# myungsub/meta-interpolation

Measured on AMD Instinct MI355X. Metric: inner-loop steps/sec, higher is better.
Workload: dtype f32 (3x3 convolutions: Winograd F(4x4) / F(2x2) on exact-f32 MFMAs, csrc/winograd4.h + winograd.hip; weight gradients and 5x5 / 7x7 / direct layers on csrc/convk*.hip: bf16x6 split operands, f32 accumulate; 51-tap op on 8-bit frames: exact integer frames x bf16x3 split taps, f32 accumulate); 1 GPU; c2_sepconv_256x448_b4_s5; plugin=sepconv, tasks_per_gpu=4, global_meta_batch=4, inner_steps=5, frame=256x448x3, inner_rule=lslr+SGD, seeded_weights=default, parallelism=task-parallel x1, 1 all-reduce of outer grads

## Files before the change

include/savfi_hip.h:

```cpp
#ifndef SAVFI_HIP_H_
#define SAVFI_HIP_H_

#include <stddef.h>
#include <stdint.h>

#ifdef __cplusplus
extern "C" {
#endif

#define SAVFI_ABI_VERSION 24

#define SAVFI_OK            0
#define SAVFI_E_NULL       (-1)
#define SAVFI_E_SHAPE      (-2)
#define SAVFI_E_UNSUPPORTED (-3)
#define SAVFI_E_TOOBIG     (-4)

int savfi_version(void);

int savfi_sepconv_fwd_f32(const float* in, const float* v, const float* h, float* out,
                          int B, int C, int Ho, int Wo, int K, void* stream);

int savfi_sepconv_bwd_f32(const float* in, const float* v, const float* h, const float* gO,
                          float* gI, float* gV, float* gH,
// ... 251 lines not shown
                              float* g1 , float* g2 , int N, int C, int H, int W, int md, void* stream);

int savfi_pwcwarp_fwd_f32(const float* img, const float* flow, float scale, float* out, int N, int C, int H, int W, void* stream);

int64_t savfi_bn_stats_scratch_floats(int N, int C, int H, int W, int n_per_group);
int savfi_bn_stats_f32(const float* x, float* mean, float* var, int64_t stat_stride, float* scratch , int N, int C, int H, int W,
                       int n_per_group, void* stream);
int savfi_bn_apply_relu_f32(const float* x, const float* mean, const float* var, int64_t stat_stride, const float* gamma ,
                            const float* beta , float eps, float* out, int N, int C, int H, int W, int n_per_group, int c_off,
                            int C_total, void* stream);
int savfi_bn_running_update_f32(int n, float* const* running, const float* const* stat, const int64_t* numel, const float* unbias,
                                float momentum, void* stream);

int savfi_maxpool2x2_f32(const float* in, float* out, int64_t planes, int H, int W, void* stream);

int savfi_upnearest2x_add_f32(const float* low, const float* skip, float* out, int64_t planes, int h, int w, int H, int W, void* stream);

int savfi_add_relu_f32(const float* a, const float* r, float* y, int64_t n, void* stream);

int savfi_charbonnier_f32(const float* a, const float* b, float* result, float* scratch, int rows, int64_t n, float eps, void* stream);
int savfi_charbonnier_bwd_f32(const float* a, const float* b, const float* g_loss, float* g_a, int rows, int64_t n, float eps,
                              void* stream);

#ifdef __cplusplus
}
#endif
#endif
```

meta-interpolation_amd/_hip.py:

```python
import ctypes
import os
import re
from ctypes import c_double, c_float, c_int, c_int64, c_void_p, POINTER

_PKG_DIR = os.path.dirname(os.path.abspath(__file__))
LIB_PATH = os.environ.get("SAVFI_HIP_LIB") or os.path.join(_PKG_DIR, "lib", "libsavfi_hip.so")
HEADER_PATH = os.path.join(os.path.dirname(_PKG_DIR), "include", "savfi_hip.h")

RULE_SGD, RULE_ADAM, RULE_ADAMAX_LSLR, RULE_ADAMAX_MSGD = 0, 1, 2, 3
LR_SCALAR, LR_ELEMENT = 0, 1
SSIM_RANGE_PER_ROW, SSIM_RANGE_BATCH, SSIM_RANGE_FIXED = 0, 1, 2
SEPCONV_PARTITION_WS, SEPCONV_PARTITION_X6, SEPCONV_PARTITION_FP32 = 0, 1, 2
ABI_VERSION = 24

_ERRORS = {-1: "SAVFI_E_NULL (a required pointer is NULL)",
           -2: "SAVFI_E_SHAPE (bad or inconsistent dimension)",
           -3: "SAVFI_E_UNSUPPORTED",
           -4: "SAVFI_E_TOOBIG (index arithmetic would overflow)"}


class SavfiHipError(RuntimeError):
    pass


# ... 116 lines not shown
    "savfi_upsample2x_window_bwd_masked_f32": [_P, _P, c_float, _P] + [c_int] * 12 + [_P],
    "savfi_upsample2x_bwd_form": [c_int, c_int, c_int],
    "savfi_bias_act_fwd_f32": [_P, _P, c_int, c_int, c_int, c_float, _P],
    "savfi_bias_act_scratch_floats": [c_int, c_int, c_int],
    "savfi_bias_act_bwd_f32": [_P, _P, _P, _P, _P, c_int, c_int, c_int, c_float, _P],
    "savfi_filterinterp_fwd_f32": [_P, _P, _P, _P] + [c_int] * 5 + [_P],
    "savfi_filterinterp_bwd_f32": [_P] * 7 + [c_int] * 5 + [_P],
    "savfi_filterinterp_fwd_slice_f32": [_P, _P, _P, _P] + [c_int] * 7 + [_P],
    "savfi_depthflowproj_scratch_bytes": [c_int, c_int, c_int],
    "savfi_depthflowproj_fwd_f32": [_P] * 5 + [c_int] * 4 + [_P],
    "savfi_depthflowproj_bwd_f32": [_P] * 7 + [c_int] * 3 + [_P],
    "savfi_correlation_fwd_f32": [_P, _P, _P] + [c_int] * 5 + [c_float, _P],
    "savfi_correlation_bwd_f32": [_P, _P, _P, _P, c_float, _P, _P] + [c_int] * 5 + [_P],
    "savfi_pwcwarp_fwd_f32": [_P, _P, c_float, _P] + [c_int] * 4 + [_P],
    "savfi_bn_stats_scratch_floats": [c_int] * 5,
    "savfi_bn_stats_f32": [_P, _P, _P, c_int64, _P] + [c_int] * 5 + [_P],
    "savfi_bn_apply_relu_f32": [_P, _P, _P, c_int64, _P, _P, c_float, _P] + [c_int] * 7 + [_P],
    "savfi_bn_running_update_f32": [c_int, _PP, _PP, _I64P, _FP, c_float, _P],
    "savfi_maxpool2x2_f32": [_P, _P, c_int64, c_int, c_int, _P],
    "savfi_upnearest2x_add_f32": [_P, _P, _P, c_int64, c_int, c_int, c_int, c_int, _P],
    "savfi_add_relu_f32": [_P, _P, _P, c_int64, _P],
    "savfi_charbonnier_f32": [_P, _P, _P, _P, c_int, c_int64, c_float, _P],
    "savfi_charbonnier_bwd_f32": [_P, _P, _P, _P, c_int, c_int64, c_float, _P],
}

_lib = None


def declared_symbols():
    with open(HEADER_PATH) as fh:
        text = fh.read()
    return sorted(set(re.findall(r"^\s*(?:int|int64_t)\s+(savfi_\w+)\s*\(", text, flags=re.M)))


def lib():
    global _lib
    if _lib is not None:
        return _lib
    if not os.path.exists(LIB_PATH):
        raise SavfiHipError(
            "%s is missing: build it with `python __graft_entry__.py build` "
            "(there is no CPU or PyTorch fallback for the savfi kernels)" % LIB_PATH)
    try:
        handle = ctypes.CDLL(LIB_PATH)
    except OSError as exc:
        raise SavfiHipError("cannot load %s: %s" % (LIB_PATH, exc))
# ... 133 lines not shown
```

meta-interpolation_amd/csrc/common.h:

```cpp
#pragma once
#include <hip/hip_runtime.h>
#include <stdint.h>
#include "savfi_hip.h"

#define SAVFI_WAVE 64


static inline int savfi_launch_status() {
  hipError_t e = hipGetLastError();
  return e == hipSuccess ? SAVFI_OK : (int)e;
}

static inline int savfi_cdiv(int64_t a, int64_t b) { return (int)((a + b - 1) / b); }

static inline int savfi_ensure_dynamic_lds(const void* kernel, size_t bytes, uint32_t& done_mask) {
  int dev = 0;
  if (hipGetDevice(&dev) != hipSuccess) return (int)hipGetLastError();
  const uint32_t bit = 1u << (dev & 31);
  if (__atomic_load_n(&done_mask, __ATOMIC_ACQUIRE) & bit) return SAVFI_OK;
  const hipError_t e = hipFuncSetAttribute(kernel, hipFuncAttributeMaxDynamicSharedMemorySize, (int)bytes);
  if (e != hipSuccess) return (int)e;
  __atomic_fetch_or(&done_mask, bit, __ATOMIC_RELEASE);
  return SAVFI_OK;
}

__device__ __forceinline__ float wave_sum(float x) {
#pragma unroll
  for (int off = 32; off > 0; off >>= 1) x += __shfl_xor(x, off, SAVFI_WAVE);
  return x;
}

template <int NW>
__device__ __forceinline__ float block_sum(float x, float* lds ) {
  x = wave_sum(x);
  const int lane = threadIdx.x & (SAVFI_WAVE - 1), wid = threadIdx.x / SAVFI_WAVE;
  if (lane == 0) lds[wid] = x;
  __syncthreads();
  float t = (threadIdx.x < NW) ? lds[threadIdx.x] : 0.f;
  if (wid == 0) t = wave_sum(t);
  __syncthreads();
  return t;
}

__device__ __forceinline__ float savfi_quantize255(float x) {
  const float v = x * 255.f;
  const float c = v < 0.f ? 0.f : (v > 255.f ? 255.f : v);
  return rintf(c);
// ... 15 lines not shown
```

meta-interpolation_amd/csrc/convk_wgrad.hip:

```cpp
#include "common.h"
#include <stdlib.h>
#include <algorithm>

typedef float f32x4 __attribute__((ext_vector_type(4)));
typedef short bf16x8 __attribute__((ext_vector_type(8)));
typedef short bf16x4 __attribute__((ext_vector_type(4)));
typedef unsigned u32x4 __attribute__((ext_vector_type(4)));
typedef int i32x4 __attribute__((ext_vector_type(4)));
__device__ float ckw_raw_buffer_load_f32(i32x4 rsrc, int voffset, int soffset, int aux) __asm("llvm.amdgcn.raw.buffer.load.f32");

namespace {

constexpr int WG_THREADS = 256;
constexpr int UR = 4, UW = 32;

__device__ __forceinline__ i32x4 ckw_rsrc(const void* base, unsigned bytes) {
  const unsigned long long p = reinterpret_cast<unsigned long long>(base);
  i32x4 r;
  r.x = (int)(unsigned)p;
  r.y = (int)(unsigned)(p >> 32);
  r.z = (int)bytes;
  r.w = 0x00020000;
  return r;
}
// ... 716 lines not shown
  a.N = N; a.T = T; a.Ci = Ci; a.Co = Co; a.H = H; a.W = W; a.pad = pad; a.reflect = reflect ? 1 : 0;
  a.Ho = H + 2 * pad - K + 1; a.Wo = W + 2 * pad - K + 1;
  a.cobs = p.cobs; a.cibs = p.cibs; a.splits = p.splits; a.units = p.units; a.units_per_split = p.ups_per_split;
  a.upr = p.upr; a.ups = p.ups;
  const int blocks = T * p.cobs * p.cibs * p.splits;
  hipStream_t st = (hipStream_t)stream;
  float* bias_partial = gb ? workspace + (size_t)p.splits * T * Co * Ci * K * K : nullptr;
  if (p.form == 2) rc = launch_wgrad3_ring(a, blocks, bias_partial, st);
  else if (K == 3 && precise) rc = p.mt == 4 ? launch_wgrad<3, 4, 1, true>(a, blocks, st) : launch_wgrad<3, 2, 1, true>(a, blocks, st);
  else if (K == 3 && p.ng == 2) rc = launch_wgrad<3, 4, 1, false, 2>(a, blocks, st);
  else if (K == 3) rc = p.mt == 4 ? launch_wgrad<3, 4, 1>(a, blocks, st) : p.nt == 2 ? launch_wgrad<3, 2, 2>(a, blocks, st) : launch_wgrad<3, 2, 1>(a, blocks, st);
  else if (K == 5) rc = precise ? launch_wgrad<5, 2, 1, true>(a, blocks, st) : p.nt == 2 ? launch_wgrad<5, 2, 2>(a, blocks, st) : launch_wgrad<5, 2, 1>(a, blocks, st);
  else rc = launch_wgrad<7, 2, 1>(a, blocks, st);
  if (rc != SAVFI_OK) return rc;
  const long long n = (long long)T * Co * Ci * K * K;
  const bool v4 = n % 4 == 0 && (((uintptr_t)workspace | (uintptr_t)gw) & 15u) == 0;
  const long long nb = gb ? (long long)T * Co : 0;
  const unsigned main_blocks = (unsigned)(v4 ? (n / 4 + 31) / 32 : (n + 31) / 32), bias_blocks = (unsigned)((nb + 31) / 32);
  if (v4) hipLaunchKernelGGL(convk_wgrad_reduce<true>, dim3(main_blocks + bias_blocks), dim3(256), 0, st, workspace, gw, n, p.splits, main_blocks, bias_partial, gb, nb);
  else hipLaunchKernelGGL(convk_wgrad_reduce<false>, dim3(main_blocks + bias_blocks), dim3(256), 0, st, workspace, gw, n, p.splits, main_blocks, bias_partial, gb, nb);
  return savfi_launch_status();
}
}
```

meta-interpolation_amd/csrc/wgrad.hip:

```cpp
#include "common.h"

namespace {

typedef float f32x4 __attribute__((ext_vector_type(4)));

constexpr int GNT = 256;
constexpr int GCO = 32, GCI = 32, GSEG = 64;
constexpr int GP = 68;
constexpr int G_FLOATS = GCO * GP;
constexpr int X_FLOATS = 3 * GCI * GP;
constexpr int BUF_FLOATS = G_FLOATS + X_FLOATS;
constexpr int TILE_FLOATS = 2 * 2 * 9 * 256;
constexpr int LDS_FLOATS_G = (2 * BUF_FLOATS > TILE_FLOATS) ? 2 * BUF_FLOATS : TILE_FLOATS;

struct WgradArgs {
  const float* x;
  const float* gz;
  float* partial;
  int Ci, Co, H, W, Ho, Wo, pad, rows, nseg, nrowchunk, cibs;
  int T;
};

struct Staged {
  float g[8], x[3][8], halo;
// ... 614 lines not shown
           bias_partial};
  if (gb) hipLaunchKernelGGL(wino_wgrad3x3<true>, dim3(p.nsplit, p.cobs * p.cibs, T), dim3(256), lds_bias, st, a);
  else hipLaunchKernelGGL(wino_wgrad3x3<false>, dim3(p.nsplit, p.cobs * p.cibs, T), dim3(256), lds, st, a);
  if (int e = savfi_launch_status()) return e;
  if (gb) {
    hipLaunchKernelGGL(wino_wgrad_bias_reduce, dim3(savfi_cdiv(Co, 64), T), dim3(64), 0, st, bias_partial, gb, Co, p.cobs, p.nsplit);
    if (int e = savfi_launch_status()) return e;
  }
  const int ntiles = p.cobs * p.cibs;
  const size_t block_floats = (size_t)ntiles * WW_BLOCK_FLOATS;
  float* stage2 = workspace + p.partial_floats;
  if (p.ngroups == 1) {
    hipLaunchKernelGGL(wino_wgrad_reduce2, dim3(savfi_cdiv(Co * Ci * 9, 256), T), dim3(256), 0, st, workspace, gw, Co, Ci, p.cibs, ntiles,
                       p.nsplit);
    return savfi_launch_status();
  }
  hipLaunchKernelGGL(wgrad_reduce1, dim3((unsigned)((block_floats / 4 + 255) / 256), p.ngroups, T), dim3(256), 0, st, workspace,
                     stage2, block_floats, p.nsplit);
  if (int e = savfi_launch_status()) return e;
  hipLaunchKernelGGL(wino_wgrad_reduce2, dim3(savfi_cdiv(Co * Ci * 9, 256), T), dim3(256), 0, st, stage2, gw, Co, Ci, p.cibs, ntiles,
                     p.ngroups);
  return savfi_launch_status();
}
```

meta-interpolation_amd/csrc/winograd.hip:

```cpp
#include "common.h"
#include <type_traits>

typedef float f32x4 __attribute__((ext_vector_type(4)));
typedef int i32x4 __attribute__((ext_vector_type(4)));
__device__ f32x4 savfi_raw_buffer_load_x4(i32x4 rsrc, int voffset, int soffset, int aux) __asm("llvm.amdgcn.raw.buffer.load.v4f32");
typedef float f32x2 __attribute__((ext_vector_type(2)));
__device__ void savfi_raw_buffer_store_x2(f32x2 data, i32x4 rsrc, int voffset, int soffset, int aux) __asm("llvm.amdgcn.raw.buffer.store.v2f32");
__device__ f32x2 savfi_raw_buffer_load_x2(i32x4 rsrc, int voffset, int soffset, int aux) __asm("llvm.amdgcn.raw.buffer.load.v2f32");
__device__ float savfi_raw_buffer_load_x1(i32x4 rsrc, int voffset, int soffset, int aux) __asm("llvm.amdgcn.raw.buffer.load.f32");
__device__ void savfi_raw_buffer_store_x1(float data, i32x4 rsrc, int voffset, int soffset, int aux) __asm("llvm.amdgcn.raw.buffer.store.f32");
__device__ void savfi_raw_buffer_store_x4(f32x4 data, i32x4 rsrc, int voffset, int soffset, int aux) __asm("llvm.amdgcn.raw.buffer.store.v4f32");

namespace {

#include "winograd4.h"

constexpr int WNT = 256;
constexpr int TILES_WG = 64;
constexpr int COB = 32;
constexpr int CIB = 4;
#ifndef WINO_VS
#define WINO_VS 80
#endif
constexpr int VS = WINO_VS;
// ... 471 lines not shown
  if (e >= total) return;
  float acc = 0.f;
  for (int s = 0; s < nsplit; ++s) acc += partial[(size_t)s * total + e];
  if (bias) {
    const size_t plane = e / HW;
    acc += bias[((plane / I) % T) * I + plane % I];
  }
  acc = acc > 0.f ? acc : slope * acc;
  if (mask) acc = mask[e] > 0.f ? acc : acc * mask_slope;
  out[e] = acc;
}

int round_up(int v, int m) { return (v + m - 1) / m * m; }

#ifndef SAVFI_WINO_SPLIT_SLOTS
#define SAVFI_WINO_SPLIT_SLOTS 512
#endif

struct WinoPlan {
  int K, I, KP, IP, off, Ho, Wo, th, tw, tile_shift, nsplit, chunks_per_split;
  int ty4, tx4;
  int64_t u_floats, partial_floats;
  bool f4;
};

inline bool f4_for(int K, int I, int form) { return form != 2 && w4::use_f4(K, I); }
inline int kp_for(int K, int I, int form) { return f4_for(K, I, form) ? w4::kp_of(K) : (K + 2 * CIB - 1) / (2 * CIB) * (2 * CIB); }
inline int ip_for(int K, int I, int form) { return f4_for(K, I, form) ? w4::ip_of(I) : (I + COB - 1) / COB * COB; }
inline int64_t u_floats_for(int K, int I, int form) { return (int64_t)(f4_for(K, I, form) ? w4::PTS : 16) * kp_for(K, I, form) * ip_for(K, I, form); }

bool make_plan(WinoPlan& p, int N, int Ci, int Co, int H, int W, int pad, int mode) {
  const int form = (mode & 2) ? 2 : 0;
  mode &= 1;
  p.K = mode == 0 ? Ci : Co;
  p.I = mode == 0 ? Co : Ci;
  p.f4 = f4_for(p.K, p.I, form);
  p.KP = kp_for(p.K, p.I, form);
  p.IP = ip_for(p.K, p.I, form);
  p.off = mode == 0 ? pad : 2 - pad;
  p.Ho = H + 2 * p.off - 2;
  p.Wo = W + 2 * p.off - 2;
  if (p.Ho <= 0 || p.Wo <= 0) return false;
  if (p.f4) {
    const int ty4 = savfi_cdiv(p.Ho, 4), tx4 = savfi_cdiv(p.Wo, 4);
    int64_t best4 = -1;
#ifndef SAVFI_W4_TS_ORDER
#define SAVFI_W4_TS_ORDER 2
// ... 2 lines not shown
    for (int s : {3, 4, 2, 5, 1, 0}) {
#elif SAVFI_W4_TS_ORDER == 1
    for (int s : {4, 3, 5, 2, 1, 0}) {
#else
    for (int s : {5, 4, 3, 2, 1, 0}) {
#endif
      const int64_t blocks = (int64_t)savfi_cdiv(ty4, w4::TT >> s) * savfi_cdiv(tx4, 1 << s);
      if (best4 < 0 || blocks < best4) { best4 = blocks; p.tile_shift = s; }
    }
    p.th = savfi_cdiv(ty4, w4::TT >> p.tile_shift);
    p.tw = savfi_cdiv(tx4, 1 << p.tile_shift);
    p.ty4 = ty4;
    p.tx4 = tx4;
    const int nchunk4 = p.KP / w4::KC;
    const int64_t wgs4 = (int64_t)p.th * p.tw * (p.IP / w4::COB) * N;
    int want4 = (int)(SAVFI_WINO_SPLIT_SLOTS / (wgs4 > 0 ? wgs4 : 1));
    want4 = (want4 < 2 || nchunk4 < 32) ? 1 : (want4 > 8 ? 8 : want4);
    int cps4 = savfi_cdiv(nchunk4, want4);
    if (cps4 < 8) cps4 = nchunk4 < 8 ? nchunk4 : 8;
    p.chunks_per_split = cps4;
    p.nsplit = savfi_cdiv(nchunk4, cps4);
    p.u_floats = u_floats_for(p.K, p.I, form);
    p.partial_floats = p.nsplit > 1 ? (int64_t)p.nsplit * N * p.I * p.Ho * p.Wo : 0;
    return true;
  }
  const int ty = savfi_cdiv(p.Ho, 2), tx = savfi_cdiv(p.Wo, 2);
  int64_t best = -1;
  for (int s : {4, 3, 5, 2}) {
    const int64_t blocks = (int64_t)savfi_cdiv(ty, TILES_WG >> s) * savfi_cdiv(tx, 1 << s);
    if (best < 0 || blocks < best) { best = blocks; p.tile_shift = s; }
  }
  p.th = savfi_cdiv(ty, TILES_WG >> p.tile_shift);
  p.tw = savfi_cdiv(tx, 1 << p.tile_shift);
  const int nchunk = p.KP / CIB;
  const int64_t wgs = (int64_t)p.th * p.tw * (p.IP / COB) * N;
  constexpr int slots = SAVFI_WINO_SPLIT_SLOTS;
  int want = (int)(slots / wgs);
  want = want < 1 ? 1 : (want > 8 ? 8 : want);
  int cps = round_up(savfi_cdiv(nchunk, want), 2);
  if (cps < 8) cps = nchunk < 8 ? nchunk : 8;
  p.chunks_per_split = cps;
  p.nsplit = savfi_cdiv(nchunk, cps);
  if (SAVFI_WINO_SPLIT_SLOTS == 0) { p.nsplit = 1; p.chunks_per_split = nchunk; }
  p.u_floats = (int64_t)16 * p.KP * p.IP;
  p.partial_floats = p.nsplit > 1 ? (int64_t)p.nsplit * N * p.I * p.Ho * p.Wo : 0;
  return true;
}



}

#ifdef WINO_TRACE
static unsigned long long* g_trace = nullptr;
static size_t g_trace_wgs = 0;
static unsigned long long* savfi_wino_trace_buffer(size_t wgs) {
  if (!g_trace) (void)hipMalloc(&g_trace, (size_t)(1 << 20) * 64);
  g_trace_wgs = wgs;
  return g_trace;
}
extern "C" int savfi_debug_wino_trace(unsigned long long* host, long long cap) {
  (void)hipDeviceSynchronize();
  const size_t n = g_trace_wgs < (size_t)cap ? g_trace_wgs : (size_t)cap;
  (void)hipMemcpy(host, g_trace, n * 64, hipMemcpyDeviceToHost);
  return (int)n;
}
#endif

// ... 16 lines not shown
static int w4_block_decode = 0;
static int64_t w4_tile_groups(const WinoPlan& p) {
  return w4_block_decode ? (int64_t)p.th * p.tw : ((int64_t)p.ty4 * p.tx4 + w4::TT - 1) / w4::TT;
}
extern "C" int64_t savfi_conv3x3_f4_launched_workgroups(int N, int Ci, int Co, int H, int W, int pad, int mode) {
  if (N <= 0 || Ci <= 0 || Co <= 0 || H <= 0 || W <= 0) return SAVFI_E_SHAPE;
  if ((mode & ~3) || (pad != 0 && pad != 1)) return SAVFI_E_UNSUPPORTED;
  WinoPlan p;
  if (!make_plan(p, N, Ci, Co, H, W, pad, mode)) return SAVFI_E_SHAPE;
  return p.f4 ? w4_tile_groups(p) * (p.IP / w4::COB) * p.nsplit * N : 0;
}
extern "C" int savfi_conv3x3_debug_f4_block_decode(int on, int* previous) {
  if (previous) *previous = w4_block_decode;
  w4_block_decode = on ? 1 : 0;
  return SAVFI_OK;
}

extern "C" int64_t savfi_conv3x3_workspace_floats(int N, int Ci, int Co, int H, int W, int pad, int mode) {
  return savfi_conv3x3_tasks_workspace_floats(N, 1, Ci, Co, H, W, pad, mode);
}

namespace {

template <int VECW, int IN16, bool MASK, bool POOL = false>
int launch_wino4(const w4::W4Args& a4, int64_t wgs4, hipStream_t st) {
  static uint32_t configured = 0;
  constexpr size_t lds4 = (size_t)w4::LDS_FLOATS * sizeof(float);
  auto kern = w4::wino4_conv3x3<VECW, IN16, MASK, POOL>;
  if (int rc = savfi_ensure_dynamic_lds(reinterpret_cast<const void*>(kern), lds4, configured)) return rc;
  hipLaunchKernelGGL(kern, dim3((unsigned)wgs4), dim3(256), lds4, st, a4);
  return savfi_launch_status();
}

bool pools_in_epilogue(const WinoPlan& p, int mode) {
  return p.f4 && (mode & 1) == 0 && p.nsplit == 1 && p.Wo % 2 == 0 && p.Ho >= 2;
}

int launch_conv(const WinoPlan& p, const float* x, const float* U, const float* bias, float* out, float* partial, int N, int T,
                int H, int W, int mode, float slope, hipStream_t st, const float* mask = nullptr, float mask_slope = 1.f,
                int out_unit16 = 0, int in_unit16 = 0, float* pooled = nullptr) {
  if (pooled && (!pools_in_epilogue(p, mode) || mask || out_unit16 || in_unit16)) return SAVFI_E_UNSUPPORTED;
  if (p.f4) {
    const int64_t ntb = w4_tile_groups(p);
    const int64_t wgs4 = ntb * (p.IP / w4::COB) * p.nsplit * N;
    if (wgs4 > 0x7fffffffLL || T > 65535) return SAVFI_E_TOOBIG;
    if (mask && (out_unit16 || in_unit16)) return SAVFI_E_UNSUPPORTED;
    if (p.nsplit > 1 && (out_unit16 || in_unit16 || !partial)) return SAVFI_E_UNSUPPORTED;
    if (in_unit16 && ((p.off != 1 && p.off != 2) || p.Wo % 2 != 0)) return SAVFI_E_UNSUPPORTED;
    w4::W4Args a4{x, U, (mode & 1) == 0 ? bias : nullptr, out, p.K, p.I, p.KP, p.IP, H, W, p.Ho, p.Wo, p.off, p.th, p.tw, slope,
                  p.tile_shift, T, N, p.nsplit > 1 ? nullptr : mask, mask_slope, out_unit16, p.nsplit, p.chunks_per_split, partial,
                  w4_block_decode ? 0 : 1, p.ty4, p.tx4, (int)ntb, p.tx4 > 1 ? (unsigned)(0x100000000ull / (unsigned)p.tx4) : 0xffffffffu,
                  pooled, p.Ho / 2, p.Wo / 2};
    const int vecw = p.Wo % 4 == 0 ? 4 : (p.Wo % 2 == 0 ? 2 : 1);
    auto go = [&](auto kern) { return kern(a4, wgs4, st); };
    if (pooled) return vecw == 4 ? go(launch_wino4<4, 0, false, true>) : go(launch_wino4<2, 0, false, true>);
    if (in_unit16 && p.off == 1) return vecw == 4 ? go(launch_wino4<4, 2, false>) : go(launch_wino4<2, 2, false>);
    if (in_unit16) return vecw == 4 ? go(launch_wino4<4, 3, false>) : go(launch_wino4<2, 3, false>);
    if (p.nsplit > 1) {
      const int rc = vecw == 4 ? go(launch_wino4<4, 0, false>) : vecw == 2 ? go(launch_wino4<2, 0, false>) : go(launch_wino4<1, 0, false>);
      if (rc != SAVFI_OK) return rc;
      const size_t total = (size_t)N * p.I * p.Ho * p.Wo;
      hipLaunchKernelGGL(wino_split_reduce, dim3((unsigned)((total + 255) / 256)), dim3(256), 0, st, partial, (mode & 1) == 0 ? bias : nullptr, out,
                         p.nsplit, total, p.I, p.Ho * p.Wo, slope, T, mask, mask_slope);
      return savfi_launch_status();
    }
    if (mask) return vecw == 4 ? go(launch_wino4<4, 0, true>) : vecw == 2 ? go(launch_wino4<2, 0, true>) : go(launch_wino4<1, 0, true>);
    return vecw == 4 ? go(launch_wino4<4, 0, false>) : vecw == 2 ? go(launch_wino4<2, 0, false>) : go(launch_wino4<1, 0, false>);
  }
  const int64_t wgs = (int64_t)p.th * p.tw * (p.IP / COB) * p.nsplit * N;
  if (wgs > 0x7fffffffLL || T > 65535) return SAVFI_E_TOOBIG;
  constexpr size_t lds = (size_t)LDS_FLOATS * sizeof(float);
  const float* b = (mode & 1) == 0 ? bias : nullptr;
  WinoArgs a{x, U, b, out, p.K, p.I, p.KP, p.IP, H, W, p.Ho, p.Wo, p.off, p.th, p.tw, slope, p.tile_shift, p.nsplit,
             p.chunks_per_split, partial, T, N, mask, mask_slope, out_unit16
#ifdef WINO_TRACE
             , savfi_wino_trace_buffer((size_t)wgs)
#endif
  };
  if (in_unit16) hipLaunchKernelGGL((wino_conv3x3<true, true>), dim3((unsigned)wgs), dim3(WNT), lds, st, a);
  else if (p.Wo % 2 == 0) hipLaunchKernelGGL(wino_conv3x3<true>, dim3((unsigned)wgs), dim3(WNT), lds, st, a);
// ... 164 lines not shown
  if (!in_unit16_ok(p, H, W)) return SAVFI_E_UNSUPPORTED;
  return launch_conv(p, gy, u, nullptr, gx, nullptr, N, T, H, W, 1, 1.f, (hipStream_t)stream, nullptr, 1.f, 0, 1);
}

extern "C" int savfi_conv3x3_dgrad_masked_form_f32(const float* gy, const float* u, const float* mask, float mask_slope, float* gx,
                                                   float* workspace, int N, int T, int Ci, int Co, int H, int W, int pad, int form,
                                                   void* stream) {
  if (!gy || !u || !gx || !mask) return SAVFI_E_NULL;
  if (form != 0 && form != 2) return SAVFI_E_UNSUPPORTED;
  WinoPlan p;
  if (int e = check_conv_args(p, N, T, Ci, Co, H, W, pad, 1 | form)) return e;
  if (p.partial_floats > 0 && !workspace) return SAVFI_E_NULL;
  return launch_conv(p, gy, u, nullptr, gx, workspace, N, T, H, W, 1, 1.f, (hipStream_t)stream, mask, mask_slope);
}
extern "C" int savfi_conv3x3_dgrad_masked_f32(const float* gy, const float* u, const float* mask, float mask_slope, float* gx,
                                              float* workspace, int N, int T, int Ci, int Co, int H, int W, int pad, void* stream) {
  return savfi_conv3x3_dgrad_masked_form_f32(gy, u, mask, mask_slope, gx, workspace, N, T, Ci, Co, H, W, pad, 0, stream);
}

extern "C" int savfi_conv3x3_f32(const float* x, const float* w, const float* bias, float* out, float* workspace,
                                 int N, int Ci, int Co, int H, int W, int pad, int mode, float slope, void* stream) {
  return savfi_conv3x3_tasks_f32(x, w, bias, out, workspace, N, 1, Ci, Co, H, W, pad, mode, slope, stream);
}
```

meta-interpolation_amd/csrc/winograd4.h:

```cpp
#pragma once

namespace w4 {

constexpr int TT = 32;
constexpr int COB = 32;
constexpr int KC = 8;
constexpr int PTS = 36;
constexpr int VBUF = PTS * KC * TT;
constexpr int XBUF = PTS * 16 * TT;
constexpr int LDS_FLOATS = XBUF > 2 * VBUF ? XBUF : 2 * VBUF;
#ifndef SAVFI_W4_MAXC
#define SAVFI_W4_MAXC 512
#endif

__host__ __device__ inline bool use_f4(int K, int I) { return K <= SAVFI_W4_MAXC && I <= SAVFI_W4_MAXC; }
__host__ __device__ inline int kp_of(int K) { return (K + KC - 1) / KC * KC; }
__host__ __device__ inline int ip_of(int I) { return (I + COB - 1) / COB * COB; }

__device__ __forceinline__ void g_rows(const float (&g)[3], float (&t)[6]) {
  const float s = g[0] + g[2];
  const float s4 = fmaf(4.f, g[2], g[0]);
  t[0] = 0.25f * g[0];
  t[1] = (s + g[1]) * (-1.f / 6.f);
  t[2] = (s - g[1]) * (-1.f / 6.f);
// ... 56 lines not shown
    float* dst = U + ((((size_t)chunk * ncob + cobq) * 4 + wv) * 2 + s2) * (18 * 64) + off;
    *reinterpret_cast<f32x4*>(dst) = *reinterpret_cast<const f32x4*>(stage + e);
  }
}

struct W4Args {
  const float* x;
  const float* U;
  const float* bias;
  float* out;
  int K, I, KP, IP, H, W, Ho, Wo, off, tiles_y, tiles_x;
  float slope;
  int tile_shift;
  int T, N;
  const float* mask;
  float mask_slope;
  int out_unit16;
  int nsplit, chunks_per_split;
  float* partial;
  int flat, ty4, tx4, ntb;
  unsigned tx_mul;
  float* pooled;
  int Hp, Wp;
};

__device__ __forceinline__ i32x4 w4_rsrc(const void* base, unsigned bytes) {
  const unsigned long long p = reinterpret_cast<unsigned long long>(base);
  i32x4 r;
  r.x = (int)(unsigned)p;
  r.y = (int)(unsigned)(p >> 32);
  r.z = (int)bytes;
  r.w = 0x00020000;
  return r;
}

__device__ __forceinline__ i32x4 w4_uniform(i32x4 r) {
  r.x = __builtin_amdgcn_readfirstlane(r.x); r.y = __builtin_amdgcn_readfirstlane(r.y);
  r.z = __builtin_amdgcn_readfirstlane(r.z); r.w = __builtin_amdgcn_readfirstlane(r.w);
  return r;
}

__device__ __forceinline__ void bt6(float d0, float d1, float d2, float d3, float d4, float d5, float (&o)[6]) {
  const float a = fmaf(-4.f, d2, d4), b = fmaf(-4.f, d1, d3);
  const float c = d4 - d2, e = d3 - d1;
  o[0] = fmaf(4.f, d0, fmaf(-5.f, d2, d4));
  o[1] = a + b;
// ... 11 lines not shown
  o[1] = a + b;
  o[2] = a - b;
  o[3] = w4_fma2(2.f, e, c);
  o[4] = w4_fma2(-2.f, e, c);
  o[5] = w4_fma2(4.f, d1, w4_fma2(-5.f, d3, d5));
}

__device__ __forceinline__ void at6(float m0, float m1, float m2, float m3, float m4, float m5, float (&o)[4]) {
  const float s1 = m1 + m2, d1 = m1 - m2, s2 = m3 + m4, d2 = m3 - m4;
  o[0] = m0 + s1 + s2;
  o[1] = fmaf(2.f, d2, d1);
  o[2] = fmaf(4.f, s2, s1);
  o[3] = fmaf(8.f, d2, d1) + m5;
}

__device__ __forceinline__ void at6p(f32x2 m0, f32x2 m1, f32x2 m2, f32x2 m3, f32x2 m4, f32x2 m5, f32x2 (&o)[4]) {
  const f32x2 s1 = m1 + m2, d1 = m1 - m2, s2 = m3 + m4, d2 = m3 - m4;
  o[0] = m0 + s1 + s2;
  o[1] = w4_fma2(2.f, d2, d1);
  o[2] = w4_fma2(4.f, s2, s1);
  o[3] = w4_fma2(8.f, d2, d1) + m5;
}

template <int VECW, int IN16, bool MASK, bool POOL = false>
__global__ __launch_bounds__(256, 2) void wino4_conv3x3(W4Args a) {
  extern __shared__ __attribute__((aligned(16))) float lds[];
  const int tid = threadIdx.x, lane = tid & 63, w = __builtin_amdgcn_readfirstlane(tid >> 6);
  const int j = lane & 15, kg = lane >> 4;

  const int nblk = a.IP / COB;
  int tb, cob, n, sp;
  {
    const unsigned flat = blockIdx.x, nwg = gridDim.x;
    const unsigned ntb = (unsigned)a.ntb;
    const unsigned xcd = flat & 7u, q8 = nwg >> 3, rem = nwg & 7u;
    unsigned item = xcd * q8 + min(xcd, rem) + (flat >> 3);
    cob = (int)(item % (unsigned)nblk);
    item /= (unsigned)nblk;
    tb = (int)(item % ntb);
    item /= ntb;
    sp = (int)(item % (unsigned)a.nsplit);
    n = (int)(item / (unsigned)a.nsplit);
  }
  const int i0 = cob * COB;
  const int task = a.T > 1 ? n % a.T : 0;
  const size_t cplane = (size_t)a.H * a.W;
  const float* xp = a.x + (size_t)n * a.K * cplane;
// ... 290 lines not shown
#pragma unroll
          for (int e = 0; e < NS; ++e) {
            if constexpr (VECW == 4) {
              const f32x4 v = savfi_raw_buffer_load_x4(mrs, (int)ooff[r][e], 0, 0);
              mk[MASK ? ch : 0][r][0] = v.x; mk[MASK ? ch : 0][r][1] = v.y; mk[MASK ? ch : 0][r][2] = v.z; mk[MASK ? ch : 0][r][3] = v.w;
            } else if constexpr (VECW == 2) {
              const f32x2 v = savfi_raw_buffer_load_x2(mrs, (int)ooff[r][e], 0, 0);
              mk[MASK ? ch : 0][r][2 * e] = v.x; mk[MASK ? ch : 0][r][2 * e + 1] = v.y;
            } else {
              mk[MASK ? ch : 0][r][e] = savfi_raw_buffer_load_x1(mrs, (int)ooff1(r, e), 0, 0);
            }
          }
      }
    }
  };
  auto by_wave = [&](auto&& f) {
    switch (w) {
      case 0: f(std::integral_constant<int, 0>{}); break;
      case 1: f(std::integral_constant<int, 1>{}); break;
      case 2: f(std::integral_constant<int, 2>{}); break;
      default: f(std::integral_constant<int, 3>{}); break;
    }
  };
  f32x2* const xl = reinterpret_cast<f32x2*>(lds) + olane;
  const float slope = a.slope;
  auto put = [&](auto cb_tag) {
    constexpr int cb = decltype(cb_tag)::value;
    by_wave([&](auto wtag) {
      constexpr int WV = decltype(wtag)::value;
#pragma unroll
      for (int q = 0; q < 9; ++q)
#pragma unroll
        for (int p = 0; p < 4; ++p)
          if (p != WV) xl[((9 * WV + q) * 4 + p) * 64] = (f32x2){acc[q][cb][p >> 1][2 * (p & 1)], acc[q][cb][p >> 1][2 * (p & 1) + 1]};
    });
  };
  auto gather = [&](auto cb_tag, f32x2 (&t4)[4][6]) {
    constexpr int cb = decltype(cb_tag)::value;
    by_wave([&](auto wtag) {
      constexpr int WV = decltype(wtag)::value;
#pragma unroll
      for (int c = 0; c < 6; ++c) {
        f32x2 m[6], o[4];
#pragma unroll
        for (int r = 0; r < 6; ++r) {
          const int xi = 6 * r + c, wp = xi / 9, q = xi % 9;
// ... 13 lines not shown
#pragma unroll
      for (int ch = 0; ch < 2; ++ch) {
        const float b = bvals[cb][ch];
        const int i = i0 + 16 * cb + 4 * okg + 2 * oh + ch;
        const i32x4 ors = w4_uniform(a.out_unit16 ? w4_rsrc(obase + (size_t)n * a.I * a.Ho * a.Wo, (unsigned)a.I * oplane) : wave_rsrc(obase, cb, ch, oplane));
        const unsigned choff = a.out_unit16 ? (i < a.I ? (unsigned)i * 64u : 0x40000000u) : 0u;
        i32x4 prs = ors;
        if constexpr (POOL) prs = w4_uniform(wave_rsrc(a.pooled, cb, ch, pplane));
        float ye[4];
#pragma unroll
        for (int r = 0; r < 4; ++r) {
          float y[4];
          at6(t4[r][0][ch], t4[r][1][ch], t4[r][2][ch], t4[r][3][ch], t4[r][4][ch], t4[r][5][ch], y);
#pragma unroll
          for (int c = 0; c < 4; ++c) {
            float v = y[c];
            if constexpr (ACT >= 1) v += b;
            if constexpr (ACT == 2) v = fmaxf(v, 0.f);
            if constexpr (ACT == 3) v = fmaxf(v, 0.f) + slope * fminf(v, 0.f);
            if constexpr (MASK) v = mk[MASK ? ch : 0][r][c] > 0.f ? v : v * a.mask_slope;
            y[c] = v;
          }
          if constexpr (VECW == 4) {
            savfi_raw_buffer_store_x4((f32x4){y[0], y[1], y[2], y[3]}, ors, (int)(ooff[r][0] + choff), 0, 0);
          } else if constexpr (VECW == 2) {
            savfi_raw_buffer_store_x2((f32x2){y[0], y[1]}, ors, (int)(ooff[r][0] + choff), 0, 0);
            savfi_raw_buffer_store_x2((f32x2){y[2], y[3]}, ors, (int)(ooff[r][1] + choff), 0, 0);
          } else {
#pragma unroll
            for (int c = 0; c < 4; ++c) savfi_raw_buffer_store_x1(y[c], ors, (int)(ooff1(r, c) + choff), 0, 0);
          }
          if constexpr (POOL) {
            if (r % 2 == 0) {
#pragma unroll
              for (int c = 0; c < 4; ++c) ye[c] = y[c];
            } else {
              const float p0 = (((ye[0] + ye[1]) + y[0]) + y[1]) / 4.f, p1 = (((ye[2] + ye[3]) + y[2]) + y[3]) / 4.f;
              if constexpr (VECW == 4) {
                savfi_raw_buffer_store_x2((f32x2){p0, p1}, prs, (int)poff[r >> 1][0], 0, 0);
              } else {
                savfi_raw_buffer_store_x1(p0, prs, (int)poff[r >> 1][0], 0, 0);
                savfi_raw_buffer_store_x1(p1, prs, (int)poff[r >> 1][PS - 1], 0, 0);
              }
            }
          }
        }
      }
    };
    if (slope == 1.f || split) {
      if (a.bias == nullptr || split) finish(std::integral_constant<int, 0>{});
      else finish(std::integral_constant<int, 1>{});
    } else if (slope == 0.f) {
      finish(std::integral_constant<int, 2>{});
    } else {
      finish(std::integral_constant<int, 3>{});
    }
  };
  using R0 = std::integral_constant<int, 0>;
  using R1 = std::integral_constant<int, 1>;
  f32x2 t4[4][6];
  fetch_mask(0);
  put(R0{});
  __syncthreads();
  gather(R0{}, t4);
  store(R0{}, t4);
  fetch_mask(1);
  __syncthreads();
  put(R1{});
  __syncthreads();
  gather(R1{}, t4);
  store(R1{}, t4);
}

}
```

Before: 253.2 inner-loop steps/sec.

## Fuse split-K partial reduction into Winograd F4 conv via ticket-based last-block combine

Adds a per-stream ticket buffer so that, when the F(4x4) Winograd conv splits the channel reduction across workgroups, the last workgroup to finish a tile sums all split partials and applies bias, activation and mask in place. This removes the separate combine kernel launch and its extra pass over the partial buffer. In exchange each workgroup now does an atomic ticket draw with fences, and the last one does a serial reduction. Stores use a cache-policy bit, and an optional pre-read mode warms the partials.

```diff
diff --git a/include/savfi_hip.h b/include/savfi_hip.h
--- a/include/savfi_hip.h
+++ b/include/savfi_hip.h
@@ -297,6 +297,15 @@
 int savfi_charbonnier_bwd_f32(const float* a, const float* b, const float* g_loss, float* g_a, int rows, int64_t n, float eps,
                               void* stream);
 
+#define SAVFI_SPLIT_FAMILY_WINO_WGRAD  0
+#define SAVFI_SPLIT_FAMILY_WINO_CONV   1
+#define SAVFI_SPLIT_FAMILY_CONVK_WGRAD 2
+int savfi_set_split_combine(int mode);
+int savfi_get_split_combine(void);
+int savfi_split_combine_prepare(void* stream);
+int savfi_split_combine_tickets(void* stream, unsigned* out, int n);
+int savfi_split_combine_form(int family, int N, int T, int Ci, int Co, int H, int W, int K, int pad, int mode, int* splits);
+
 #ifdef __cplusplus
 }
 #endif
diff --git a/meta-interpolation_amd/_hip.py b/meta-interpolation_amd/_hip.py
--- a/meta-interpolation_amd/_hip.py
+++ b/meta-interpolation_amd/_hip.py
@@ -162,6 +162,11 @@
     "savfi_add_relu_f32": [_P, _P, _P, c_int64, _P],
     "savfi_charbonnier_f32": [_P, _P, _P, _P, c_int, c_int64, c_float, _P],
     "savfi_charbonnier_bwd_f32": [_P, _P, _P, _P, c_int, c_int64, c_float, _P],
+    "savfi_set_split_combine": [c_int],
+    "savfi_get_split_combine": [],
+    "savfi_split_combine_prepare": [_P],
+    "savfi_split_combine_tickets": [_P, _P, c_int],
+    "savfi_split_combine_form": [c_int] * 10 + [_P],
 }
 
 _lib = None
diff --git a/meta-interpolation_amd/csrc/common.h b/meta-interpolation_amd/csrc/common.h
--- a/meta-interpolation_amd/csrc/common.h
+++ b/meta-interpolation_amd/csrc/common.h
@@ -23,6 +23,90 @@
   __atomic_fetch_or(&done_mask, bit, __ATOMIC_RELEASE);
   return SAVFI_OK;
 }
+
+constexpr int SAVFI_TICKET_WORDS = 1 << 16;
+unsigned* savfi_split_combine_acquire(hipStream_t st, int* mode);
+void savfi_split_combine_launch_failed(hipStream_t st);
+int savfi_wino_wgrad_combine_form(int N, int T, int Ci, int Co, int H, int W, int pad, int* splits);
+int savfi_wino_conv_combine_form(int N, int T, int Ci, int Co, int H, int W, int pad, int mode, int* splits);
+int savfi_convk_wgrad_combine_form(int N, int T, int Ci, int Co, int H, int W, int K, int pad, int* splits);
+
+#ifdef __HIPCC__
+__device__ __forceinline__ bool savfi_ticket_draw(unsigned* tickets, unsigned tile, unsigned splits, unsigned* flag) {
+  asm volatile("s_waitcnt vmcnt(0)" ::: "memory");
+  __syncthreads();
+  if (threadIdx.x == 0) {
+    const unsigned drawn = __hip_atomic_fetch_add(tickets + tile, 1u, __ATOMIC_RELAXED, __HIP_MEMORY_SCOPE_AGENT);
+    const unsigned last = drawn == splits - 1u ? 1u : 0u;
+    if (last) {
+      __builtin_amdgcn_fence(__ATOMIC_ACQUIRE, "agent");
+      asm volatile("s_waitcnt vmcnt(0)" ::: "memory");
+    }
+    *flag = last;
+  }
+  __syncthreads();
+  return __builtin_amdgcn_readfirstlane(*reinterpret_cast<volatile unsigned*>(flag)) != 0u;
+}
+template <int V, int NI, typename BiasOf>
+__device__ __forceinline__ void savfi_split_finish_rows(const float* partial, size_t total, int nsplit, const unsigned (&e)[NI], unsigned ok,
+                                                        BiasOf&& bias_of, bool has_bias, float slope, const float* mask, float mask_slope,
+                                                        float* out, bool write) {
+  typedef float fv __attribute__((ext_vector_type(V)));
+  fv acc[NI];
+#pragma unroll
+  for (int k = 0; k < NI; ++k) acc[k] = (fv)(0.f);
+  int s = 0;
+  for (; s + 1 < nsplit; s += 2) {
+    const float* p0 = partial + (size_t)s * total;
+    const float* p1 = p0 + total;
+    fv v0[NI], v1[NI];
+#pragma unroll
+    for (int k = 0; k < NI; ++k) v0[k] = *reinterpret_cast<const fv*>(p0 + e[k]);
+#pragma unroll
+    for (int k = 0; k < NI; ++k) v1[k] = *reinterpret_cast<const fv*>(p1 + e[k]);
+#pragma unroll
+    for (int k = 0; k < NI; ++k) acc[k] += v0[k];
+#pragma unroll
+    for (int k = 0; k < NI; ++k) acc[k] += v1[k];
+  }
+  if (s < nsplit) {
+    const float* p0 = partial + (size_t)s * total;
+    fv v0[NI];
+#pragma unroll
+    for (int k = 0; k < NI; ++k) v0[k] = *reinterpret_cast<const fv*>(p0 + e[k]);
+#pragma unroll
+    for (int k = 0; k < NI; ++k) acc[k] += v0[k];
+  }
+  if (!write) {
+#pragma unroll
+    for (int k = 0; k < NI; ++k)
+#pragma unroll
+      for (int q = 0; q < V; ++q) asm volatile("" ::"v"(acc[k][q]));
+    return;
+  }
+  fv mv[NI];
+  if (mask) {
+#pragma unroll
+    for (int k = 0; k < NI; ++k) mv[k] = *reinterpret_cast<const fv*>(mask + e[k]);
+  }
+#pragma unroll
+  for (int k = 0; k < NI; ++k) {
+    const float b = has_bias ? bias_of(k) : 0.f;
+#pragma unroll
+    for (int q = 0; q < V; ++q) {
+      float a = acc[k][q];
+      if (has_bias) a += b;
+      a = a > 0.f ? a : slope * a;
+      if (mask) a = mv[k][q] > 0.f ? a : a * mask_slope;
+      acc[k][q] = a;
+    }
+    if (ok >> k & 1u) *reinterpret_cast<fv*>(out + e[k]) = acc[k];
+  }
+}
+__device__ __forceinline__ void savfi_ticket_reset(unsigned* tickets, unsigned tile) {
+  if (threadIdx.x == 0) __hip_atomic_store(tickets + tile, 0u, __ATOMIC_RELAXED, __HIP_MEMORY_SCOPE_AGENT);
+}
+#endif
 
 __device__ __forceinline__ float wave_sum(float x) {
 #pragma unroll
diff --git a/meta-interpolation_amd/csrc/convk_wgrad.hip b/meta-interpolation_amd/csrc/convk_wgrad.hip
--- a/meta-interpolation_amd/csrc/convk_wgrad.hip
+++ b/meta-interpolation_amd/csrc/convk_wgrad.hip
@@ -762,3 +762,11 @@
   return savfi_launch_status();
 }
 }
+
+int savfi_convk_wgrad_combine_form(int N, int T, int Ci, int Co, int H, int W, int K, int pad, int* splits) {
+  WgPlan p;
+  const int rc = wg_plan(p, N, T, Ci, Co, H, W, K, pad, false);
+  if (rc != SAVFI_OK) return rc;
+  *splits = p.splits;
+  return 0;
+}
diff --git a/meta-interpolation_amd/csrc/split_combine.hip b/meta-interpolation_amd/csrc/split_combine.hip
--- /dev/null
+++ b/meta-interpolation_amd/csrc/split_combine.hip
@@ -0,0 +1,125 @@
+#include "common.h"
+#include <mutex>
+#include <vector>
+
+#ifndef SAVFI_SPLIT_COMBINE
+#define SAVFI_SPLIT_COMBINE 1
+#endif
+
+namespace {
+
+struct TicketBlock {
+  int dev;
+  hipStream_t stream;
+  unsigned* words;
+  bool dirty;
+};
+std::mutex g_lock;
+std::vector<TicketBlock> g_blocks;
+int g_mode = SAVFI_SPLIT_COMBINE;
+
+bool stream_is_capturing(hipStream_t st) {
+  hipStreamCaptureStatus cs = hipStreamCaptureStatusNone;
+  if (hipStreamIsCapturing(st, &cs) != hipSuccess) { (void)hipGetLastError(); return true; }
+  return cs != hipStreamCaptureStatusNone;
+}
+
+TicketBlock* find_block(int dev, hipStream_t st) {
+  for (TicketBlock& b : g_blocks)
+    if (b.dev == dev && b.stream == st) return &b;
+  return nullptr;
+}
+
+unsigned* block_for(hipStream_t st) {
+  int dev = 0;
+  if (hipGetDevice(&dev) != hipSuccess) { (void)hipGetLastError(); return nullptr; }
+  TicketBlock* b = find_block(dev, st);
+  if (b && !b->dirty) return b->words;
+  if (stream_is_capturing(st)) return nullptr;
+  if (!b) {
+    unsigned* words = nullptr;
+    if (hipMalloc(reinterpret_cast<void**>(&words), (size_t)SAVFI_TICKET_WORDS * sizeof(unsigned)) != hipSuccess) {
+      (void)hipGetLastError();
+      return nullptr;
+    }
+    g_blocks.push_back(TicketBlock{dev, st, words, true});
+    b = &g_blocks.back();
+  }
+  if (hipMemsetAsync(b->words, 0, (size_t)SAVFI_TICKET_WORDS * sizeof(unsigned), st) != hipSuccess) {
+    (void)hipGetLastError();
+    return nullptr;
+  }
+  b->dirty = false;
+  return b->words;
+}
+
+}
+
+unsigned* savfi_split_combine_acquire(hipStream_t st, int* mode) {
+  std::lock_guard<std::mutex> hold(g_lock);
+  *mode = g_mode;
+  return g_mode == 0 ? nullptr : block_for(st);
+}
+
+void savfi_split_combine_launch_failed(hipStream_t st) {
+  std::lock_guard<std::mutex> hold(g_lock);
+  int dev = 0;
+  if (hipGetDevice(&dev) != hipSuccess) { (void)hipGetLastError(); return; }
+  if (TicketBlock* b = find_block(dev, st)) b->dirty = true;
+}
+
+extern "C" int savfi_set_split_combine(int mode) {
+  if (mode < 0 || mode > 2) return SAVFI_E_UNSUPPORTED;
+  std::lock_guard<std::mutex> hold(g_lock);
+  g_mode = mode;
+  return SAVFI_OK;
+}
+
+extern "C" int savfi_get_split_combine(void) {
+  std::lock_guard<std::mutex> hold(g_lock);
+  return g_mode;
+}
+
+extern "C" int savfi_split_combine_prepare(void* stream) {
+  std::lock_guard<std::mutex> hold(g_lock);
+  return block_for((hipStream_t)stream) ? SAVFI_OK : SAVFI_E_UNSUPPORTED;
+}
+
+extern "C" int savfi_split_combine_tickets(void* stream, unsigned* out, int n) {
+  if (!out) return SAVFI_E_NULL;
+  if (n <= 0 || n > SAVFI_TICKET_WORDS) return SAVFI_E_SHAPE;
+  hipStream_t st = (hipStream_t)stream;
+  unsigned* words = nullptr;
+  {
+    std::lock_guard<std::mutex> hold(g_lock);
+    int dev = 0;
+    if (hipGetDevice(&dev) != hipSuccess) return (int)hipGetLastError();
+    if (TicketBlock* b = find_block(dev, st)) words = b->words;
+  }
+  if (!words) return SAVFI_E_UNSUPPORTED;
+  if (hipMemcpyAsync(out, words, (size_t)n * sizeof(unsigned), hipMemcpyDeviceToHost, st) != hipSuccess) return (int)hipGetLastError();
+  if (hipStreamSynchronize(st) != hipSuccess) return (int)hipGetLastError();
+  return SAVFI_OK;
+}
+
+extern "C" int savfi_split_combine_form(int family, int N, int T, int Ci, int Co, int H, int W, int K, int pad, int mode, int* splits) {
+  int sp = 0;
+  int rc;
+  switch (family) {
+    case SAVFI_SPLIT_FAMILY_WINO_WGRAD:
+      if (K != 3) return SAVFI_E_UNSUPPORTED;
+      rc = savfi_wino_wgrad_combine_form(N, T, Ci, Co, H, W, pad, &sp);
+      break;
+    case SAVFI_SPLIT_FAMILY_WINO_CONV:
+      if (K != 3) return SAVFI_E_UNSUPPORTED;
+      rc = savfi_wino_conv_combine_form(N, T, Ci, Co, H, W, pad, mode, &sp);
+      break;
+    case SAVFI_SPLIT_FAMILY_CONVK_WGRAD:
+      rc = savfi_convk_wgrad_combine_form(N, T, Ci, Co, H, W, K, pad, &sp);
+      break;
+    default:
+      return SAVFI_E_UNSUPPORTED;
+  }
+  if (rc >= 0 && splits) *splits = sp;
+  return rc;
+}
diff --git a/meta-interpolation_amd/csrc/wgrad.hip b/meta-interpolation_amd/csrc/wgrad.hip
--- a/meta-interpolation_amd/csrc/wgrad.hip
+++ b/meta-interpolation_amd/csrc/wgrad.hip
@@ -660,3 +660,12 @@
                      p.ngroups);
   return savfi_launch_status();
 }
+
+int savfi_wino_wgrad_combine_form(int N, int T, int Ci, int Co, int H, int W, int pad, int* splits) {
+  if (N <= 0 || T <= 0 || N % T != 0 || Ci <= 0 || Co <= 0 || H <= 0 || W <= 0) return SAVFI_E_SHAPE;
+  if (pad != 0 && pad != 1) return SAVFI_E_UNSUPPORTED;
+  WWPlan p;
+  if (!ww_plan(p, N, T, Ci, Co, H, W, pad)) return SAVFI_E_SHAPE;
+  *splits = p.nsplit;
+  return 0;
+}
diff --git a/meta-interpolation_amd/csrc/winograd.hip b/meta-interpolation_amd/csrc/winograd.hip
--- a/meta-interpolation_amd/csrc/winograd.hip
+++ b/meta-interpolation_amd/csrc/winograd.hip
@@ -517,7 +517,16 @@
   int ty4, tx4;
   int64_t u_floats, partial_floats;
   bool f4;
+  bool combine;
 };
+
+#ifndef SAVFI_WINO4_COMBINE_KB
+#define SAVFI_WINO4_COMBINE_KB 128
+#endif
+inline bool wino_combines(bool f4, int nsplit, int64_t tiles, int64_t out_floats) {
+  return f4 && nsplit > 1 && (int64_t)nsplit * 64 <= SAVFI_WINO4_COMBINE_KB && tiles <= SAVFI_TICKET_WORDS &&
+         out_floats < ((int64_t)1 << 31);
+}
 
 inline bool f4_for(int K, int I, int form) { return form != 2 && w4::use_f4(K, I); }
 inline int kp_for(int K, int I, int form) { return f4_for(K, I, form) ? w4::kp_of(K) : (K + 2 * CIB - 1) / (2 * CIB) * (2 * CIB); }
@@ -566,6 +575,7 @@
     p.nsplit = savfi_cdiv(nchunk4, cps4);
     p.u_floats = u_floats_for(p.K, p.I, form);
     p.partial_floats = p.nsplit > 1 ? (int64_t)p.nsplit * N * p.I * p.Ho * p.Wo : 0;
+    p.combine = wino_combines(true, p.nsplit, wgs4, (int64_t)N * p.I * p.Ho * p.Wo);
     return true;
   }
   const int ty = savfi_cdiv(p.Ho, 2), tx = savfi_cdiv(p.Wo, 2);
@@ -588,6 +598,7 @@
   if (SAVFI_WINO_SPLIT_SLOTS == 0) { p.nsplit = 1; p.chunks_per_split = nchunk; }
   p.u_floats = (int64_t)16 * p.KP * p.IP;
   p.partial_floats = p.nsplit > 1 ? (int64_t)p.nsplit * N * p.I * p.Ho * p.Wo : 0;
+  p.combine = wino_combines(false, p.nsplit, wgs, (int64_t)N * p.I * p.Ho * p.Wo);
   return true;
 }
 
@@ -650,11 +661,11 @@
 
 namespace {
 
-template <int VECW, int IN16, bool MASK, bool POOL = false>
+template <int VECW, int IN16, bool MASK, bool POOL = false, bool COMBINE = false>
 int launch_wino4(const w4::W4Args& a4, int64_t wgs4, hipStream_t st) {
   static uint32_t configured = 0;
   constexpr size_t lds4 = (size_t)w4::LDS_FLOATS * sizeof(float);
-  auto kern = w4::wino4_conv3x3<VECW, IN16, MASK, POOL>;
+  auto kern = w4::wino4_conv3x3<VECW, IN16, MASK, POOL, COMBINE>;
   if (int rc = savfi_ensure_dynamic_lds(reinterpret_cast<const void*>(kern), lds4, configured)) return rc;
   hipLaunchKernelGGL(kern, dim3((unsigned)wgs4), dim3(256), lds4, st, a4);
   return savfi_launch_status();
@@ -678,12 +689,23 @@
     w4::W4Args a4{x, U, (mode & 1) == 0 ? bias : nullptr, out, p.K, p.I, p.KP, p.IP, H, W, p.Ho, p.Wo, p.off, p.th, p.tw, slope,
                   p.tile_shift, T, N, p.nsplit > 1 ? nullptr : mask, mask_slope, out_unit16, p.nsplit, p.chunks_per_split, partial,
                   w4_block_decode ? 0 : 1, p.ty4, p.tx4, (int)ntb, p.tx4 > 1 ? (unsigned)(0x100000000ull / (unsigned)p.tx4) : 0xffffffffu,
-                  pooled, p.Ho / 2, p.Wo / 2};
+                  pooled, p.Ho / 2, p.Wo / 2, nullptr, mask, 0};
     const int vecw = p.Wo % 4 == 0 ? 4 : (p.Wo % 2 == 0 ? 2 : 1);
     auto go = [&](auto kern) { return kern(a4, wgs4, st); };
     if (pooled) return vecw == 4 ? go(launch_wino4<4, 0, false, true>) : go(launch_wino4<2, 0, false, true>);
     if (in_unit16 && p.off == 1) return vecw == 4 ? go(launch_wino4<4, 2, false>) : go(launch_wino4<2, 2, false>);
     if (in_unit16) return vecw == 4 ? go(launch_wino4<4, 3, false>) : go(launch_wino4<2, 3, false>);
+    if (p.nsplit > 1 && p.combine && ((((uintptr_t)partial | (uintptr_t)out | (uintptr_t)mask) & 15u) == 0)) {
+      int cmode = 0;
+      a4.tickets = savfi_split_combine_acquire(st, &cmode);
+      if (a4.tickets) {
+        a4.pre_read = cmode == 2;
+        const int rc = vecw == 4 ? go(launch_wino4<4, 0, false, false, true>)
+                                 : vecw == 2 ? go(launch_wino4<2, 0, false, false, true>) : go(launch_wino4<1, 0, false, false, true>);
+        if (rc > 0) savfi_split_combine_launch_failed(st);
+        return rc;
+      }
+    }
     if (p.nsplit > 1) {
       const int rc = vecw == 4 ? go(launch_wino4<4, 0, false>) : vecw == 2 ? go(launch_wino4<2, 0, false>) : go(launch_wino4<1, 0, false>);
       if (rc != SAVFI_OK) return rc;
@@ -894,3 +916,10 @@
                                  int N, int Ci, int Co, int H, int W, int pad, int mode, float slope, void* stream) {
   return savfi_conv3x3_tasks_f32(x, w, bias, out, workspace, N, 1, Ci, Co, H, W, pad, mode, slope, stream);
 }
+
+int savfi_wino_conv_combine_form(int N, int T, int Ci, int Co, int H, int W, int pad, int mode, int* splits) {
+  WinoPlan p;
+  if (int rc = check_conv_args(p, N, T, Ci, Co, H, W, pad, mode)) return rc;
+  *splits = p.nsplit;
+  return p.combine ? 1 : 0;
+}
diff --git a/meta-interpolation_amd/csrc/winograd4.h b/meta-interpolation_amd/csrc/winograd4.h
--- a/meta-interpolation_amd/csrc/winograd4.h
+++ b/meta-interpolation_amd/csrc/winograd4.h
@@ -102,6 +102,9 @@
   unsigned tx_mul;
   float* pooled;
   int Hp, Wp;
+  unsigned* tickets;
+  const float* rmask;
+  int pre_read;
 };
 
 __device__ __forceinline__ i32x4 w4_rsrc(const void* base, unsigned bytes) {
@@ -159,7 +162,7 @@
   o[3] = w4_fma2(8.f, d2, d1) + m5;
 }
 
-template <int VECW, int IN16, bool MASK, bool POOL = false>
+template <int VECW, int IN16, bool MASK, bool POOL = false, bool COMBINE = false>
 __global__ __launch_bounds__(256, 2) void wino4_conv3x3(W4Args a) {
   extern __shared__ __attribute__((aligned(16))) float lds[];
   const int tid = threadIdx.x, lane = tid & 63, w = __builtin_amdgcn_readfirstlane(tid >> 6);
@@ -496,6 +499,7 @@
       default: f(std::integral_constant<int, 3>{}); break;
     }
   };
+  constexpr int OAUX = COMBINE ? 16 : 0;
   f32x2* const xl = reinterpret_cast<f32x2*>(lds) + olane;
   const float slope = a.slope;
   auto put = [&](auto cb_tag) {
@@ -555,13 +559,13 @@
             y[c] = v;
           }
           if constexpr (VECW == 4) {
-            savfi_raw_buffer_store_x4((f32x4){y[0], y[1], y[2], y[3]}, ors, (int)(ooff[r][0] + choff), 0, 0);
+            savfi_raw_buffer_store_x4((f32x4){y[0], y[1], y[2], y[3]}, ors, (int)(ooff[r][0] + choff), 0, OAUX);
           } else if constexpr (VECW == 2) {
-            savfi_raw_buffer_store_x2((f32x2){y[0], y[1]}, ors, (int)(ooff[r][0] + choff), 0, 0);
-            savfi_raw_buffer_store_x2((f32x2){y[2], y[3]}, ors, (int)(ooff[r][1] + choff), 0, 0);
+            savfi_raw_buffer_store_x2((f32x2){y[0], y[1]}, ors, (int)(ooff[r][0] + choff), 0, OAUX);
+            savfi_raw_buffer_store_x2((f32x2){y[2], y[3]}, ors, (int)(ooff[r][1] + choff), 0, OAUX);
           } else {
 #pragma unroll
-            for (int c = 0; c < 4; ++c) savfi_raw_buffer_store_x1(y[c], ors, (int)(ooff1(r, c) + choff), 0, 0);
+            for (int c = 0; c < 4; ++c) savfi_raw_buffer_store_x1(y[c], ors, (int)(ooff1(r, c) + choff), 0, OAUX);
           }
           if constexpr (POOL) {
             if (r % 2 == 0) {
@@ -603,6 +607,37 @@
   __syncthreads();
   gather(R1{}, t4);
   store(R1{}, t4);
-}
-
-}
+  if constexpr (COMBINE) {
+    const size_t total = (size_t)a.N * a.I * a.Ho * a.Wo;
+    constexpr int UPR = 4 / VECW, UNITS = COB * TT * 4 * UPR, NI = VECW == 4 ? 8 : 16;
+    static_assert(UNITS % (256 * NI) == 0, "whole batches");
+    auto finish_tile = [&](bool write) {
+#pragma unroll 1
+      for (int u0 = tid; u0 < UNITS; u0 += 256 * NI) {
+        unsigned e[NI], ok = 0;
+        auto channel = [&](int k) { return i0 + (u0 + 256 * k) / (UPR * 4 * TT); };
+#pragma unroll
+        for (int k = 0; k < NI; ++k) {
+          const int u = u0 + 256 * k, col = u % UPR, rest = u / UPR;
+          const int slot = rest & (TT - 1), r = (rest / TT) & 3, i = channel(k);
+          int ty, tx;
+          const bool on = tile_of(tbo, slot, ty, tx);
+          const int y = 4 * ty + r, x = 4 * tx + VECW * col;
+          const bool in = on && i < a.I && y < a.Ho && x < a.Wo;
+          ok |= in ? 1u << k : 0u;
+          e[k] = in ? (unsigned)(((n * a.I + i) * a.Ho + y) * a.Wo + x) : 0u;
+        }
+        savfi_split_finish_rows<VECW, NI>(a.partial, total, a.nsplit, e, ok, [&](int k) { return a.bias[task * a.I + min(channel(k), a.I - 1)]; },
+                                          a.bias != nullptr, a.slope, a.rmask, a.mask_slope, a.out, write);
+      }
+    };
+    const unsigned tile = ((unsigned)n * (unsigned)a.ntb + (unsigned)tbo) * (unsigned)nblk + (unsigned)cob;
+    if (a.pre_read) finish_tile(false);
+    if (savfi_ticket_draw(a.tickets, tile, (unsigned)a.nsplit, reinterpret_cast<unsigned*>(lds))) {
+      finish_tile(true);
+      savfi_ticket_reset(a.tickets, tile);
+    }
+  }
+}
+
+}
```

After: 253.1 inner-loop steps/sec. Within noise of the previous version (-0.0%).
